# patflick/psac

Hardware: AMD Instinct MI355X
Metric: MChars/s SA+LCP build; rank-pair radix-sort HBM GB/s vs peak (higher is better)
Workload: dtype u64

## Files before the change

include/psacx.h:

```cpp
#ifndef PSACX_H
#define PSACX_H

#include <stddef.h>
#include <stdint.h>

#ifdef __cplusplus
extern "C" {
#endif

typedef struct psacx_ctx psacx_ctx;

enum {
    PSACX_OK = 0,
    PSACX_EINVAL = -1,
    PSACX_ERANGE = -2,
    PSACX_ENOMEM = -3,
    PSACX_EHIP = -4,
    PSACX_EDEVICE = -5,
    PSACX_ENOGPU = -6
};

enum {
    PSACX_LCP = 1u,
    PSACX_NO_FAST = 2u,
// ... 20 lines not shown
    double ms_total;
    double ms_alphabet, ms_kmer, ms_sort_hist, ms_sort_scatter, ms_rebucket, ms_isa_scatter,
           ms_gather, ms_compact, ms_rmq_build, ms_finalize;
    double ms_sort_scatter3, ms_sort_tilehist, ms_sort_scatter2;
    uint64_t scatter_launches[3];
    uint64_t scatter_records[3];
    uint64_t scatter_bytes[3];
    uint64_t hist_bytes;
    uint64_t workspace_bytes;
    uint64_t onew_passes;
    uint64_t heavy_rounds;
    uint64_t heavy_records;
    uint64_t light_records;
    uint64_t level_gathers;
    double ms_host[9];
} psacx_stats;


#define PSACX_STREAM_DEFAULT ((void*)(intptr_t)-1)
int psacx_create(psacx_ctx** out, int device, void* stream);
void psacx_destroy(psacx_ctx* ctx);
const char* psacx_strerror(int code);
const char* psacx_last_hip_error(const psacx_ctx* ctx);
int psacx_trim(psacx_ctx* ctx);

enum {
    PSACX_OPT_RESET = 0, PSACX_OPT_FORCE_DIET, PSACX_OPT_DIET_CAP, PSACX_OPT_ONE_STAGE, PSACX_OPT_TIES_RADIX, PSACX_OPT_NO_ONE_WORD,
    PSACX_OPT_ONE_WORD_ALWAYS, PSACX_OPT_ONE_WORD_MIN, PSACX_OPT_WIDEN_LAST, PSACX_OPT_NO_DIGIT_BYTES, PSACX_OPT_NO_BUCKET_SORT,
    PSACX_OPT_ISA_UPDATE, PSACX_OPT_GATHER, PSACX_OPT_NO_HEAVY, PSACX_OPT_NO_WHOLE, PSACX_OPT_NO_LAZY_RANKS, PSACX_OPT_NO_EARLY_OUT, PSACX_OPT_COUNT
};
int psacx_configure(psacx_ctx* ctx, int option, uint64_t value);
int psacx_configure_from_env(psacx_ctx* ctx);
const char* psacx_debug_env(const char* name);

int psacx_construct_u32(psacx_ctx* ctx, const uint8_t* text, uint64_t n, uint32_t k,
                        uint32_t flags, uint32_t* SA, uint32_t* ISA, uint32_t* LCP);
int psacx_construct_u64(psacx_ctx* ctx, const uint8_t* text, uint64_t n, uint32_t k,
                        uint32_t flags, uint64_t* SA, uint64_t* ISA, uint64_t* LCP);
int psacx_construct_dev_u32(psacx_ctx* ctx, const uint8_t* d_text, uint64_t n, uint32_t k,
                            uint32_t flags, uint32_t* d_SA, uint32_t* d_ISA, uint32_t* d_LCP);
int psacx_construct_dev_u64(psacx_ctx* ctx, const uint8_t* d_text, uint64_t n, uint32_t k,
                            uint32_t flags, uint64_t* d_SA, uint64_t* d_ISA, uint64_t* d_LCP);

int psacx_construct_lc_u32(psacx_ctx* ctx, const uint8_t* text, uint64_t n, uint32_t k, uint32_t flags,
// ... 147 lines not shown
```

psac_amd/_lib.py:

```python
import ctypes as C
import os

_HERE = os.path.dirname(os.path.abspath(__file__))
LIB_PATH = os.path.join(_HERE, "lib", "libpsacx.so")

PSACX_LCP = 1
PSACX_NO_FAST = 2
PSACX_PROFILE = 4
PSACX_MAX_ROUNDS = 72

OPTIONS = {"reset": 0, "force_diet": 1, "diet_cap": 2, "one_stage": 3, "ties_radix": 4, "no_one_word": 5, "one_word_always": 6, "one_word_min": 7,
           "widen_last": 8, "no_digit_bytes": 9, "no_bucket_sort": 10, "isa_update": 11, "gather": 12, "no_heavy": 13, "no_whole": 14, "no_lazy_ranks": 15, "no_early_out": 16}
MULTI_OPTIONS = {"layout": 1, "slab": 2, "output_slack": 3, "trace": 4, "wire_piece": 5, "pieces": 6, "check_chunks": 7, "global_refine_sort": 8,
                 "one_stage": 9, "two_word": 10, "one_word": 11, "no_slices": 12, "slice_wide": 13, "slice_shape": 14}
MULTI_FORCE_WIRE, MULTI_NO_RCCL, MULTI_SHM = 1, 2, 4
ENV_KNOBS = bool(os.environ.get("PSACX_ENV_KNOBS"))
if ENV_KNOBS and os.environ.get("PSACX_LIB"):
    LIB_PATH = os.environ["PSACX_LIB"]

EXPORTS = [
    "psacx_create", "psacx_destroy", "psacx_strerror", "psacx_last_hip_error", "psacx_trim", "psacx_configure", "psacx_configure_from_env", "psacx_debug_env",
    "psacx_construct_u32", "psacx_construct_u64", "psacx_construct_dev_u32", "psacx_construct_dev_u64",
    "psacx_construct_gsa_u32", "psacx_construct_gsa_u64", "psacx_construct_gsa_dev_u32", "psacx_construct_gsa_dev_u64",
    "psacx_construct_lc_u32", "psacx_construct_lc_u64", "psacx_construct_lc_dev_u32", "psacx_construct_lc_dev_u64",
    "psacx_get_stats", "psacx_profile", "psacx_check_dev_u32", "psacx_check_dev_u64", "psacx_check_gsa_dev_u32", "psacx_check_gsa_dev_u64", "psacx_pair_sort_dev_u32", "psacx_pair_sort_dev_u64", "psacx_ansv_u32",
    "psacx_ansv_u64", "psacx_ansv_dev_u32", "psacx_ansv_dev_u64", "psacx_suffix_tree_u32", "psacx_suffix_tree_u64", "psacx_dev_alloc", "psacx_dev_free", "psacx_copy_h2d", "psacx_copy_d2h", "psacx_sync",
    "psacx_rand_dna", "psacx_synth_text_dev",
# ... 13 lines not shown
                ("unfinished_elements", C.c_uint64), ("sort_passes", C.c_uint32),
                ("sort_passes_skipped", C.c_uint32)]


class Stats(C.Structure):
    _fields_ = [("sigma", C.c_uint32), ("bits_per_char", C.c_uint32), ("k", C.c_uint32),
                ("n_rounds", C.c_uint32), ("rounds", Round * PSACX_MAX_ROUNDS),
                ("ms_total", C.c_double), ("ms_alphabet", C.c_double), ("ms_kmer", C.c_double),
                ("ms_sort_hist", C.c_double), ("ms_sort_scatter", C.c_double), ("ms_rebucket", C.c_double),
                ("ms_isa_scatter", C.c_double), ("ms_gather", C.c_double), ("ms_compact", C.c_double),
                ("ms_rmq_build", C.c_double), ("ms_finalize", C.c_double),
                ("ms_sort_scatter3", C.c_double), ("ms_sort_tilehist", C.c_double), ("ms_sort_scatter2", C.c_double),
                ("scatter_launches", C.c_uint64 * 3), ("scatter_records", C.c_uint64 * 3),
                ("scatter_bytes", C.c_uint64 * 3), ("hist_bytes", C.c_uint64), ("workspace_bytes", C.c_uint64), ("onew_passes", C.c_uint64),
                ("heavy_rounds", C.c_uint64), ("heavy_records", C.c_uint64), ("light_records", C.c_uint64), ("level_gathers", C.c_uint64),
                ("ms_host", C.c_double * 9)]


class PsacxError(RuntimeError):
    def __init__(self, code, msg):
        RuntimeError.__init__(self, "psacx error %d: %s" % (code, msg))
        self.code = code


_lib = None


def load():
    global _lib
    if _lib is not None:
        return _lib
# ... 109 lines not shown
```

psac_amd/csrc/construct.hpp:

```cpp
#pragma once
#include <chrono>
#include <thread>
#include "engine.hpp"
#include "bucket_sort.hpp"
#include "heavy_keys.hpp"

namespace psacx {

constexpr int SCAN_ITEMS = 8;
#ifndef RB1W_BLOCK
#define RB1W_BLOCK 512
#endif
template <typename T> struct ScanCfg {
    static constexpr int BLOCK = sizeof(T) == 8 ? 512 : 768;
    static constexpr int TILE = BLOCK * SCAN_ITEMS;
};
constexpr int SCAN_TILE_MIN = 512 * SCAN_ITEMS;

constexpr unsigned SCAN_CHUNKS = 4096, SCAN_CHUNK = 1024 * 4;
template <typename T> struct Work {
    T *bsa;
    SortBufs<T> x, y;
    SortBufs<T> ry;
    T *pos_a, *pos_b;
// ... 571 lines not shown
                               reinterpret_cast<unsigned*>(w.sc.d_desc + 256), (int)lo1);
        } else
            hipLaunchKernelGGL((key_pairs_kernel<T, KB, KI>), dim3((unsigned)nb), dim3(KB), 0, c->stream, d_text, n, n,
                               tab, ks, first_in.k1, k2rec, w.sc.d_partials, (const T*)nullptr);
        PSACX_HIP(c, hipGetLastError());
        PSACX_TRY(summary_finish(c, w.sc, (unsigned)nb));
        return PSACX_OK;
    };
    if (!one_word) PSACX_TRY(make_keys(hist_in_keys));

    std::memset(r0, 0, sizeof(*r0));
    if (two_stage) {
        SortBufs<T> in1{first_in.k1, nullptr, first_in.v}, alt1{first_alt.k1, nullptr, first_alt.v};
        bool packed1 = false;
        uint8_t* tie_bytes = nullptr;
        onew_recs = false;
        if constexpr (sizeof(T) == 8) {
            if (one_word) {
                uint64_t* s1 = nullptr;
                const bool keep = !kn.widen_last && !kn.ties_radix && isa_narrow_levels<T>(n, kn) > 0;
                uint8_t* const dig = kn.no_digit_bytes ? (uint8_t*)nullptr : reinterpret_cast<uint8_t*>(w.diet ? w.x.k2 : first_alt.k2);
                tie_bytes = (keep && !kn.no_digit_bytes) ? reinterpret_cast<uint8_t*>(w.diet ? w.y.k2 : first_in.k2) : (uint8_t*)nullptr;
                const int rc1 = prefix_sort_1w(c, w.sc, reinterpret_cast<uint64_t*>(in1.k1), reinterpret_cast<uint64_t*>(alt1.k1),
                                               reinterpret_cast<uint64_t*>(d_sa), n, lo1, lead, r0, &s1, d_text, n, tab, ks, !kn.one_word_always,
                                               keep ? &onew_view : nullptr, dig,
                                               (in1.k1 == w.x.k1 && onew_pad_total<T>(n)) ? ONEW_PAD : (uint64_t)0, tie_bytes);
                if (rc1 == PSACX_RETRY_1STAGE) {
                    two_stage = false; retry_one_stage = true; one_word = false;
                } else if (rc1 == PSACX_RETRY_1W) {
                    one_word = false;
                    PSACX_TRY(make_keys(hist_in_keys));
                }
                else {
                    PSACX_TRY(rc1);
                    sorted.k1 = reinterpret_cast<T*>(s1); sorted.k2 = nullptr; sorted.v = d_sa;
                    packed1 = true;
                    onew_recs = keep;
                }
            }
        } else one_word = false;
        if (retry_one_stage) continue;
        if (!one_word)
        PSACX_TRY(pair_sort<T>(c, w.sc, in1, alt1, n, true, bits_w1, 0, w.diet ? (T*)nullptr : d_sa, &sorted, r0,
                               ks.spec, n, true, lo1, hist_in_keys ? (int)lo1 : -1));
        if (w.diet && sorted.v != d_sa)
            PSACX_HIP(c, hipMemcpyAsync(d_sa, sorted.v, n * sizeof(T), hipMemcpyDeviceToDevice, c->stream));
        T* S1 = sorted.k1;
        T* const S2 = w.diet ? w.x.k2 : first_alt.k2;
        T* free_k1 = (S1 == w.x.k1) ? w.y.k1 : w.x.k1;
        constexpr int TB = 256, TI = sizeof(T) == 8 ? 32 : 16, TG = 8;
        unsigned long long* d_big = reinterpret_cast<unsigned long long*>(w.d_totals + 2);
        unsigned long long* h_big = reinterpret_cast<unsigned long long*>(c->pinned + 64);
        {
            ProfScope ps(c, TC_GATHER);
            PSACX_HIP(c, hipMemsetAsync(d_big, 0, sizeof(unsigned long long), c->stream));
            const uint64_t nb = (n + (uint64_t)TB * TI - 1) / ((uint64_t)TB * TI);
            if constexpr (sizeof(T) == 8) {
                if (onew_recs)
                    hipLaunchKernelGGL((tie_resolve_1w_kernel<TB, TI, TG>), dim3((unsigned)nb), dim3(TB), 0, c->stream, reinterpret_cast<uint64_t*>(S1),
                                       reinterpret_cast<uint64_t*>(free_k1), reinterpret_cast<uint64_t*>(S2), n, onew_view, d_text, n, tab, ks, d_big,
                                       (const uint8_t*)tie_bytes);
            }
            if (!kn.ties_radix && !onew_recs)
                hipLaunchKernelGGL((tie_resolve_kernel<T, TB, TI, TG>), dim3((unsigned)nb), dim3(TB), 0, c->stream, S1, d_sa, S2, n, lo1,
                                   d_text, n, tab, ks, d_big, packed1);
            PSACX_HIP(c, hipGetLastError());
        }
        PSACX_HIP(c, hipMemcpyAsync(h_big, d_big, sizeof(unsigned long long), hipMemcpyDeviceToHost, c->stream));
        PSACX_HIP(c, hipStreamSynchronize(c->stream));
        if constexpr (sizeof(T) == 8) {
            if (onew_recs && *h_big) {
                ProfScope ps(c, TC_GATHER);
                hipLaunchKernelGGL(onew_widen_kernel<0>, dim3(grid_for(c, n, 256, 8)), dim3(256), 0, c->stream, reinterpret_cast<const uint64_t*>(S1), n, onew_view,
                                   reinterpret_cast<uint64_t*>(free_k1), reinterpret_cast<uint64_t*>(d_sa));
                PSACX_HIP(c, hipGetLastError());
                std::swap(S1, free_k1);
                sorted.k1 = S1;
                onew_recs = false;
            }
        }
        if (*h_big || kn.ties_radix) {
            const uint64_t ntiles = (n + ScanCfg<T>::TILE - 1) / ScanCfg<T>::TILE;
            {
                ProfScope ps(c, TC_COMPACT);
                hipLaunchKernelGGL((count_active_kernel<T, ScanCfg<T>::BLOCK, SCAN_ITEMS>), dim3((unsigned)ntiles), dim3(ScanCfg<T>::BLOCK), 0,
// ... 639 lines not shown
```

psac_amd/csrc/engine.hpp:

```cpp
#pragma once
#include <hip/hip_runtime.h>

#include <algorithm>
#include <cstdio>
#include <cstdlib>
#include <cstring>
#include <condition_variable>
#include <functional>
#include <map>
#include <mutex>
#include <string>
#include <thread>
#include <sched.h>
#include <pthread.h>
#include <cctype>
#include <cstdio>
#include <vector>

#include "../../include/psacx.h"
#include "radix.hpp"
#include "sa_kernels.hpp"

namespace psacx {

// ... 11 lines not shown
    bool force_diet = false;
    uint64_t diet_cap = 0;
    bool one_stage = false;
    bool ties_radix = false;
    bool no_one_word = false;
    bool one_word_always = false;
    unsigned one_word_min = 24;
    int isa_update = 0;
    bool no_digit_bytes = false;
    bool no_bucket_sort = false;
    int gather = 0;
    bool no_heavy = false;
    bool no_early_out = false;
    bool no_lazy_ranks = false;
    bool no_whole = false;
    bool widen_last = false;
};

}

struct psacx_ctx {
    int device = 0;
    hipStream_t stream = nullptr;
    bool own_stream = false;
    char* slab = nullptr;
    size_t slab_bytes = 0;
    char* aux = nullptr;
    size_t aux_bytes = 0;
    char* pinned = nullptr;
    char* pinned_dev = nullptr;
// ... 781 lines not shown
            if (w != dst) PSACX_HIP(c, hipMemcpyAsync(dst, w, n * sizeof(T), hipMemcpyDeviceToDevice, c->stream));
        } else if (dst != cur.v) {
            PSACX_HIP(c, hipMemcpyAsync(dst, cur.v, n * sizeof(T), hipMemcpyDeviceToDevice, c->stream));
        }
        cur.v = dst;
    }
    *res = cur;
    return PSACX_OK;
}

constexpr int PSACX_RETRY_1W = 1001;
constexpr int PSACX_RETRY_1STAGE = 1002;
#ifndef PSACX_1W_ITEMS
#define PSACX_1W_ITEMS 8
#endif
struct OneWordLayout { unsigned slab; uint64_t total_slabs, vtiles; size_t hist_bytes, slab_bytes, tabs_bytes, need; };
template <int TILE>
inline OneWordLayout onew_layout(unsigned long long* h_tabs, uint64_t ntiles_hint) {
    OneWordLayout lay;
    lay.slab = ntiles_hint >= (1u << 16) ? 64u : 16u;
    uint64_t total_slabs = 0;
    for (int d = 0; d < RADIX; ++d) {
        const uint64_t cnt = h_tabs[d + 1] - h_tabs[d];
        h_tabs[RADIX + 1 + d] = total_slabs;
        total_slabs += ((cnt + TILE - 1) / TILE + lay.slab - 1) / lay.slab;
    }
    h_tabs[2 * RADIX + 1] = total_slabs;
    lay.total_slabs = total_slabs;
    lay.vtiles = total_slabs * lay.slab;
    lay.hist_bytes = ((size_t)lay.vtiles * RADIX * sizeof(unsigned) + 255) & ~(size_t)255;
    lay.slab_bytes = ((size_t)total_slabs * RADIX * sizeof(unsigned long long) + 255) & ~(size_t)255;
    lay.tabs_bytes = (2 * (RADIX + 1) * sizeof(unsigned long long) + 64 + total_slabs * sizeof(SlabInfo) + 255) & ~(size_t)255;
    lay.need = 256 + lay.hist_bytes + lay.slab_bytes + (size_t)RADIX * RADIX * 8 + lay.tabs_bytes;
    return lay;
}
inline int onew_bucket_passes(psacx_ctx* c, char* scratch, const unsigned long long* h_tabs, const OneWordLayout& lay, uint64_t* cur, uint64_t* oth, uint64_t* sa_out,
                              unsigned sfield, unsigned low, unsigned lo1, uint64_t nrec, uint64_t** s1, OneWordView* view_out = nullptr, uint8_t* dig = nullptr,
                              uint64_t in_pad = 0, uint8_t* tie_bytes = nullptr) {
    constexpr int BLOCK = 512, ITEMS_B = PSACX_1W_ITEMS, TILE = BLOCK * ITEMS_B;
    unsigned* tile_hist = reinterpret_cast<unsigned*>(scratch + 256);
    unsigned long long* slab_tot = reinterpret_cast<unsigned long long*>(scratch + 256 + lay.hist_bytes);
    unsigned long long* base2 = reinterpret_cast<unsigned long long*>(scratch + 256 + lay.hist_bytes + lay.slab_bytes);
    unsigned long long* d_tabs = base2 + (size_t)RADIX * RADIX;
    OneWordTabs tb;
    tb.bucket_off = d_tabs; tb.slab_start = d_tabs + RADIX + 1; tb.slab = lay.slab;
    SlabInfo* slab_info = reinterpret_cast<SlabInfo*>((reinterpret_cast<uintptr_t>(d_tabs + 2 * (RADIX + 1)) + 31) & ~(uintptr_t)31);
    tb.slab_info = slab_info;
    *s1 = cur;
    if (view_out) { view_out->off = d_tabs; view_out->low = low; view_out->sfield = sfield; view_out->lo1 = lo1; }
    PSACX_HIP(c, hipMemcpyAsync(d_tabs, h_tabs, 2 * (RADIX + 1) * sizeof(unsigned long long), hipMemcpyHostToDevice, c->stream));
    if (lay.total_slabs == 0) return PSACX_OK;
    const uint64_t total_slabs = lay.total_slabs, vtiles = lay.vtiles;
    hipLaunchKernelGGL(radix_slab_info_kernel<0>, dim3((unsigned)((total_slabs + 255) / 256)), dim3(256), 0, c->stream, tb.bucket_off, tb.slab_start,
                       (unsigned)total_slabs, (unsigned)(lay.slab * TILE), slab_info);
    PSACX_HIP(c, hipGetLastError());
    const int npass = (int)((low + RADIX_BITS - 1) / RADIX_BITS);
    for (int j = 0; j < npass; ++j) {
        const bool last = j + 1 == npass;
        const int shift = (int)sfield + j * RADIX_BITS;
        {
            ProfScope ps(c, TC_SORT_TILEHIST);
            if (dig && j > 0) hipLaunchKernelGGL((radix_tile_hist_bytes_kernel<BLOCK, ITEMS_B>), dim3((unsigned)((vtiles + BLOCK / WAVE - 1) / (BLOCK / WAVE))), dim3(BLOCK), 0, c->stream,
                                                 (const uint8_t*)dig, tb, (unsigned)vtiles, tile_hist);
            else
            hipLaunchKernelGGL((radix_tile_hist1w_kernel<BLOCK, ITEMS_B>), dim3((unsigned)vtiles), dim3(BLOCK), 0, c->stream, (const uint64_t*)cur, tb, shift, tile_hist,
                               j == 0 ? in_pad : (uint64_t)0);
            hipLaunchKernelGGL(radix_slab_scan1w_kernel<0>, dim3((unsigned)total_slabs), dim3(RADIX), 0, c->stream, tile_hist, tb, (unsigned)TILE, slab_tot);
            hipLaunchKernelGGL(radix_top_scan1w_kernel<0>, dim3(RADIX), dim3(RADIX), 0, c->stream, slab_tot, tb, base2);
            PSACX_HIP(c, hipGetLastError());
        }
        ProfScope ps(c, TC_SORT_SCATTER2);
        PSACX_HIP(c, hipMemsetAsync(scratch, 0, 256, c->stream));
        if (!last || view_out)
            hipLaunchKernelGGL((radix_scatter1w_kernel<BLOCK, ITEMS_B, 8>), dim3((unsigned)vtiles), dim3(BLOCK), 0, c->stream, (const uint64_t*)cur, oth, (uint64_t*)nullptr, shift,
                               tb, base2, tile_hist, slab_tot, reinterpret_cast<unsigned*>(scratch), sort_chunk_for(nrec, true), 0u,
                               last ? tie_bytes : dig, last ? (int)sfield : shift + RADIX_BITS, j == 0 ? in_pad : (uint64_t)0);
        else {
            hipLaunchKernelGGL((radix_scatter1w_kernel<BLOCK, ITEMS_B, 9>), dim3((unsigned)vtiles), dim3(BLOCK), 0, c->stream, (const uint64_t*)cur, oth, sa_out, shift,
                               tb, base2, tile_hist, slab_tot, reinterpret_cast<unsigned*>(scratch), sort_chunk_for(nrec, true), lo1 | (low << 8) | (sfield << 16),
                               (uint8_t*)nullptr, 0, j == 0 ? in_pad : (uint64_t)0);
        }
        PSACX_HIP(c, hipGetLastError());
        c->stats.scatter_launches[2] += 1; c->stats.scatter_records[2] += nrec; c->stats.scatter_bytes[2] += ((last && !view_out ? 24ull : 16ull) + (((dig && !last) || (last && view_out && tie_bytes)) ? 1ull : 0ull)) * nrec;
        c->stats.onew_passes += 1;
        std::swap(cur, oth);
    }
    *s1 = cur;
    return PSACX_OK;
}
inline int prefix_sort_1w(psacx_ctx* c, SortScratch& sc, uint64_t* k0, uint64_t* a, uint64_t* sa_out, uint64_t n, unsigned lo1, unsigned lead,
                          psacx_round* rs, uint64_t** s1, const uint8_t* text, uint64_t n_text, const CodeTable& tab, const KeyShape& ks, bool probe,
                          OneWordView* view_out = nullptr, uint8_t* dig = nullptr, uint64_t pad = 0, uint8_t* tie_bytes = nullptr) {
    constexpr int BLOCK = 512, ITEMS = 8, TILE0 = BLOCK * ITEMS;
    constexpr int TILE = BLOCK * PSACX_1W_ITEMS;
    const unsigned low = lead - RADIX_BITS;
    const unsigned sfield = 64 - low;
    const uint64_t ntiles = (n + TILE0 - 1) / TILE0;
    char* const scratch = sc.d_desc;
    const unsigned slab0 = slab_tiles_for(ntiles);
    const uint64_t nslabs0 = (ntiles + slab0 - 1) / slab0;
    unsigned* tile_hist0 = reinterpret_cast<unsigned*>(scratch + 256);
    unsigned long long* slab_tot0 = reinterpret_cast<unsigned long long*>(scratch + 256 + ((ntiles * RADIX * sizeof(unsigned) + 255) & ~(size_t)255));
    unsigned long long* base0 = sc.d_base;
    {
        ProfScope ps(c, TC_KMER);
        const uint64_t stride = std::max<uint64_t>(64, n >> 20), samples = n / stride;
        uint64_t slots = 1; while (slots < 4 * samples) slots <<= 1;
// ... 22 lines not shown
    PSACX_HIP(c, hipStreamSynchronize(c->stream));
    unsigned long long* h_tabs = sc.h_base + RADIX;
    for (int d = 0; d < RADIX; ++d) h_tabs[d] = sc.h_base[d];
    h_tabs[RADIX] = n;
    const OneWordLayout lay = onew_layout<TILE>(h_tabs, ntiles);
    if (lay.need > sc.desc_bytes || lay.vtiles >= (1ull << 31)) return PSACX_RETRY_1W;
    {
        ProfScope ps(c, TC_KMER);
        PSACX_HIP(c, hipMemsetAsync(scratch, 0, 256, c->stream));
        hipLaunchKernelGGL((key_scatter1w_kernel<BLOCK, ITEMS>), dim3((unsigned)ntiles), dim3(BLOCK), 0, c->stream, text, n, n_text, tab, ks, pad ? k0 : a, (int)(lo1 + low),
                           base0, tile_hist0, slab_tot0, reinterpret_cast<unsigned*>(scratch), sort_chunk_for(n, true), slab0, lo1 | (sfield << 16), (uint64_t)0,
                           (uint8_t*)nullptr, 0, pad);
        PSACX_HIP(c, hipGetLastError());
    }
    uint64_t* cur = nullptr;
    if (pad) PSACX_TRY(onew_bucket_passes(c, scratch, h_tabs, lay, k0, a, sa_out, sfield, low, lo1, n, &cur, view_out, dig, pad, tie_bytes));
    else PSACX_TRY(onew_bucket_passes(c, scratch, h_tabs, lay, a, k0, sa_out, sfield, low, lo1, n, &cur, view_out, dig, 0, tie_bytes));
    *s1 = cur;
    if (rs) { rs->sort_passes = (uint32_t)((low + RADIX_BITS - 1) / RADIX_BITS + 1); rs->sort_passes_skipped = 0; }
    return PSACX_OK;
}

}
```

psac_amd/csrc/psacx_abi.hip:

```cpp
#include "engine.hpp"

namespace psacx {
int construct_dev_u32(psacx_ctx*, const uint8_t*, uint64_t, uint32_t, uint32_t, uint32_t*, uint32_t*, uint32_t*);
int construct_dev_u64(psacx_ctx*, const uint8_t*, uint64_t, uint32_t, uint32_t, uint64_t*, uint64_t*, uint64_t*);
int construct_host_u32(psacx_ctx*, const uint8_t*, uint64_t, uint32_t, uint32_t, uint32_t*, uint32_t*, uint32_t*);
int construct_gsa_host_u32(psacx_ctx*, const uint8_t*, uint64_t, const uint64_t*, uint64_t, uint32_t, uint32_t, uint32_t*, uint32_t*, uint32_t*);
int construct_gsa_dev_u32(psacx_ctx*, const uint8_t*, uint64_t, const uint64_t*, uint64_t, uint32_t, uint32_t, uint32_t*, uint32_t*, uint32_t*);
int construct_gsa_host_u64(psacx_ctx*, const uint8_t*, uint64_t, const uint64_t*, uint64_t, uint32_t, uint32_t, uint64_t*, uint64_t*, uint64_t*);
int construct_gsa_dev_u64(psacx_ctx*, const uint8_t*, uint64_t, const uint64_t*, uint64_t, uint32_t, uint32_t, uint64_t*, uint64_t*, uint64_t*);
int construct_lc_host_u32(psacx_ctx*, const uint8_t*, uint64_t, uint32_t, uint32_t, uint32_t*, uint32_t*, uint32_t*, uint8_t*);
int construct_lc_host_u64(psacx_ctx*, const uint8_t*, uint64_t, uint32_t, uint32_t, uint64_t*, uint64_t*, uint64_t*, uint8_t*);
int construct_lc_dev_u32(psacx_ctx*, const uint8_t*, uint64_t, uint32_t, uint32_t, uint32_t*, uint32_t*, uint32_t*, uint8_t*);
int construct_lc_dev_u64(psacx_ctx*, const uint8_t*, uint64_t, uint32_t, uint32_t, uint64_t*, uint64_t*, uint64_t*, uint8_t*);
int construct_host_u64(psacx_ctx*, const uint8_t*, uint64_t, uint32_t, uint32_t, uint64_t*, uint64_t*, uint64_t*);
int pair_sort_dev_u32(psacx_ctx*, uint32_t*, uint32_t*, uint32_t*, uint64_t, uint32_t);
int pair_sort_dev_u64(psacx_ctx*, uint64_t*, uint64_t*, uint64_t*, uint64_t, uint32_t);
int check_dev_u32(psacx_ctx*, const uint8_t*, uint64_t, const uint32_t*, const uint32_t*, const uint32_t*, uint64_t*);
int check_dev_u64(psacx_ctx*, const uint8_t*, uint64_t, const uint64_t*, const uint64_t*, const uint64_t*, uint64_t*);
int check_gsa_dev_u32(psacx_ctx*, const uint8_t*, uint64_t, const uint64_t*, uint64_t, const uint32_t*, const uint32_t*, const uint32_t*, uint64_t*);
int check_gsa_dev_u64(psacx_ctx*, const uint8_t*, uint64_t, const uint64_t*, uint64_t, const uint64_t*, const uint64_t*, const uint64_t*, uint64_t*);
int synth_text_dev(psacx_ctx*, uint8_t*, uint64_t, uint64_t, int, uint64_t, uint64_t);
int suffix_tree_host_u32(psacx_ctx*, const uint8_t*, uint64_t, const uint32_t*, const uint32_t*, uint64_t*, uint32_t*);
int suffix_tree_host_u64(psacx_ctx*, const uint8_t*, uint64_t, const uint64_t*, const uint64_t*, uint64_t*, uint32_t*);
int ansv_host_u32(psacx_ctx*, const uint32_t*, uint64_t, int, int, uint64_t, uint64_t*, uint64_t*);
// ... 78 lines not shown
    case PSACX_OPT_DIET_CAP: k.diet_cap = value; return PSACX_OK;
    case PSACX_OPT_ONE_STAGE: k.one_stage = value != 0; return PSACX_OK;
    case PSACX_OPT_TIES_RADIX: k.ties_radix = value != 0; return PSACX_OK;
    case PSACX_OPT_NO_ONE_WORD: k.no_one_word = value != 0; return PSACX_OK;
    case PSACX_OPT_ONE_WORD_ALWAYS: k.one_word_always = value != 0; return PSACX_OK;
    case PSACX_OPT_ONE_WORD_MIN: if (value > 62) return PSACX_EINVAL; k.one_word_min = value ? (unsigned)std::max<uint64_t>(16, value) : 24u; return PSACX_OK;
    case PSACX_OPT_WIDEN_LAST: k.widen_last = value != 0; return PSACX_OK;
    case PSACX_OPT_NO_DIGIT_BYTES: k.no_digit_bytes = value != 0; return PSACX_OK;
    case PSACX_OPT_NO_BUCKET_SORT: k.no_bucket_sort = value != 0; return PSACX_OK;
    case PSACX_OPT_ISA_UPDATE: if (value > 2) return PSACX_EINVAL; k.isa_update = (int)value; return PSACX_OK;
    case PSACX_OPT_GATHER: if (value > 2) return PSACX_EINVAL; k.gather = (int)value; return PSACX_OK;
    case PSACX_OPT_NO_HEAVY: k.no_heavy = value != 0; return PSACX_OK;
    case PSACX_OPT_NO_WHOLE: k.no_whole = value != 0; return PSACX_OK;
    case PSACX_OPT_NO_LAZY_RANKS: k.no_lazy_ranks = value != 0; return PSACX_OK;
    case PSACX_OPT_NO_EARLY_OUT: k.no_early_out = value != 0; return PSACX_OK;
    default: return PSACX_EINVAL;
    }
}

const char* psacx_debug_env(const char* name) { return name ? getenv(name) : nullptr; }

int psacx_configure_from_env(psacx_ctx* c) {
    if (!c) return PSACX_EINVAL;
    static const struct { const char* name; int option; } flags[] = {
        {"PSACX_FORCE_DIET", PSACX_OPT_FORCE_DIET}, {"PSACX_ONE_STAGE", PSACX_OPT_ONE_STAGE}, {"PSACX_TIES_RADIX", PSACX_OPT_TIES_RADIX},
        {"PSACX_NO_ONE_WORD", PSACX_OPT_NO_ONE_WORD}, {"PSACX_ONE_WORD_ALWAYS", PSACX_OPT_ONE_WORD_ALWAYS}, {"PSACX_WIDEN_LAST", PSACX_OPT_WIDEN_LAST},
        {"PSACX_NO_DIGIT_BYTES", PSACX_OPT_NO_DIGIT_BYTES}, {"PSACX_NO_BUCKET_SORT", PSACX_OPT_NO_BUCKET_SORT}, {"PSACX_NO_HEAVY", PSACX_OPT_NO_HEAVY},
        {"PSACX_NO_WHOLE", PSACX_OPT_NO_WHOLE}, {"PSACX_NO_LAZY_RANKS", PSACX_OPT_NO_LAZY_RANKS},
        {"PSACX_NO_EARLY_OUT", PSACX_OPT_NO_EARLY_OUT}};
    (void)psacx_configure(c, PSACX_OPT_RESET, 0);
    for (const auto& f : flags) if (psacx_debug_env(f.name)) (void)psacx_configure(c, f.option, 1);
    if (const char* e = psacx_debug_env("PSACX_DIET_CAP")) (void)psacx_configure(c, PSACX_OPT_DIET_CAP, strtoull(e, nullptr, 10));
    if (const char* e = psacx_debug_env("PSACX_ONE_WORD_MIN")) (void)psacx_configure(c, PSACX_OPT_ONE_WORD_MIN, strtoull(e, nullptr, 10));
    if (const char* e = psacx_debug_env("PSACX_ISA_UPDATE")) (void)psacx_configure(c, PSACX_OPT_ISA_UPDATE, e[0] == 's' ? 1 : 2);
    if (const char* e = psacx_debug_env("PSACX_GATHER")) (void)psacx_configure(c, PSACX_OPT_GATHER, e[0] == 'f' ? 1 : 2);
    return PSACX_OK;
}

int psacx_trim(psacx_ctx* c) {
    if (!c) return PSACX_EINVAL;
    PSACX_HIP(c, hipSetDevice(c->device));
    PSACX_HIP(c, hipStreamSynchronize(c->stream));
    if (c->slab) { PSACX_HIP(c, hipFree(c->slab)); c->slab = nullptr; c->slab_bytes = 0; }
    if (c->aux) { PSACX_HIP(c, hipFree(c->aux)); c->aux = nullptr; c->aux_bytes = 0; }
    if (c->io) { PSACX_HIP(c, hipFree(c->io)); c->io = nullptr; c->io_bytes = 0; }
    if (c->dstage) { PSACX_HIP(c, hipFree(c->dstage)); c->dstage = nullptr; }
    for (int i = 0; i < psacx_ctx::STAGE_SLOTS; ++i) {
// ... 145 lines not shown
```

psac_amd/csrc/sa_kernels.hpp:

```cpp
#pragma once
#ifndef RB_WAVES_ATTR
#define RB_WAVES_ATTR
#endif
#ifndef RB_ABLATE
#define RB_ABLATE 0
#endif
#include <type_traits>
#include "dev_common.hpp"

namespace psacx {

constexpr int RADIX_P = 256;

struct CodeTable { uint16_t c[256]; };

template <typename T>
__device__ __forceinline__ void key_summary_add(unsigned long long* partials, T or1, T and1, T or2, T and2) {
    __shared__ unsigned long long red[4][16];
    or1 = wave_reduce<T>(or1, OpOr()); and1 = wave_reduce<T>(and1, OpAnd());
    or2 = wave_reduce<T>(or2, OpOr()); and2 = wave_reduce<T>(and2, OpAnd());
    const unsigned wave = threadIdx.x / WAVE, nw = (blockDim.x + WAVE - 1) / WAVE;
    const unsigned long long hi = ~(unsigned long long)(T)~(T)0;
    if (lane_id() == 0) {
        red[0][wave] = (unsigned long long)or1; red[1][wave] = (unsigned long long)and1 | hi;
// ... 1518 lines not shown
        }
        unsigned rank = 0;
#pragma unroll
        for (int j = 0; j < G; ++j) {
            const T o1 = shfl<T>(k1, (int)(seg0 + j)), o2 = shfl<T>(k2, (int)(seg0 + j));
            if (o1 < k1 || (o1 == k1 && (o2 < k2 || (o2 == k2 && (unsigned)j < m)))) ++rank;
        }
        const bool moved = ((unsigned)(__ballot(member && rank != m) >> seg0) & ((1u << G) - 1u)) != 0;
        if (member) {
            W1[e + rank] = k1; S2[e + rank] = k2;
            if (moved) R[e + rank] = (key << ow.sfield) | sa;
        }
    }
}

template <typename T, int BLOCK>
__global__ __launch_bounds__(BLOCK) void gather_prefix_ties_kernel(uint64_t cnt, T* __restrict__ K1, const T* __restrict__ V,
                                          const uint8_t* __restrict__ text, uint64_t n_text, CodeTable tab, KeyShape ks,
                                          T* __restrict__ K2, unsigned long long* __restrict__ summary, bool packed = false,
                                          const uint32_t* __restrict__ ord = nullptr, unsigned lo1 = 0, int v32 = 0) {
    __shared__ uint16_t ctab[256];
    for (int i = threadIdx.x; i < 256; i += BLOCK) ctab[i] = tab.c[i];
    __syncthreads();
    const uint64_t stride = (uint64_t)gridDim.x * blockDim.x;
    const T lowmask = lo1 ? (T)(((T)1 << lo1) - 1) : (T)0;
    T o1 = 0, a1 = ~(T)0, o2 = 0, a2 = ~(T)0;
    for (uint64_t j = (uint64_t)blockIdx.x * blockDim.x + threadIdx.x; j < cnt; j += stride) {
        T k1 = K1[j], k2;
        const uint64_t sa = v32 ? (uint64_t)reinterpret_cast<const uint32_t*>(V)[j] : (uint64_t)V[j];
        if (packed && ord) window_low_and_word2<T>(text, n_text, ctab, ks, sa, k1, lo1, k1, k2);
// ... 548 lines not shown
```

Baseline: 24730.

## Skip last one-word radix pass and order short runs locally in tie kernel

In the one-word prefix sort, the final (lowest) radix digit pass is skipped when local ordering is enabled. Records sharing the higher digits are instead ordered inside a new tile-local kernel that insertion-sorts short runs in shared memory and fuses this with tie resolution. Runs that are too long are appended to a list and sorted by a separate per-run counting-sort kernel. The goal is to save one full global scatter pass over the records. In exchange it adds a host round trip for the long-run count, and falls back to a one-stage retry if the list overflows its cap.

```diff
diff --git a/include/psacx.h b/include/psacx.h
--- a/include/psacx.h
+++ b/include/psacx.h
@@ -58,6 +58,8 @@
     uint64_t light_records;
     uint64_t level_gathers;
     double ms_host[9];
+    uint64_t local_long_runs;
+    uint64_t local_list_overflows;
 } psacx_stats;
 
 
@@ -71,7 +73,8 @@
 enum {
     PSACX_OPT_RESET = 0, PSACX_OPT_FORCE_DIET, PSACX_OPT_DIET_CAP, PSACX_OPT_ONE_STAGE, PSACX_OPT_TIES_RADIX, PSACX_OPT_NO_ONE_WORD,
     PSACX_OPT_ONE_WORD_ALWAYS, PSACX_OPT_ONE_WORD_MIN, PSACX_OPT_WIDEN_LAST, PSACX_OPT_NO_DIGIT_BYTES, PSACX_OPT_NO_BUCKET_SORT,
-    PSACX_OPT_ISA_UPDATE, PSACX_OPT_GATHER, PSACX_OPT_NO_HEAVY, PSACX_OPT_NO_WHOLE, PSACX_OPT_NO_LAZY_RANKS, PSACX_OPT_NO_EARLY_OUT, PSACX_OPT_COUNT
+    PSACX_OPT_ISA_UPDATE, PSACX_OPT_GATHER, PSACX_OPT_NO_HEAVY, PSACX_OPT_NO_WHOLE, PSACX_OPT_NO_LAZY_RANKS, PSACX_OPT_NO_EARLY_OUT,
+    PSACX_OPT_NO_LOCAL_ORDER, PSACX_OPT_LOCAL_LIST_CAP, PSACX_OPT_COUNT
 };
 int psacx_configure(psacx_ctx* ctx, int option, uint64_t value);
 int psacx_configure_from_env(psacx_ctx* ctx);
diff --git a/psac_amd/_lib.py b/psac_amd/_lib.py
--- a/psac_amd/_lib.py
+++ b/psac_amd/_lib.py
@@ -10,7 +10,8 @@
 PSACX_MAX_ROUNDS = 72
 
 OPTIONS = {"reset": 0, "force_diet": 1, "diet_cap": 2, "one_stage": 3, "ties_radix": 4, "no_one_word": 5, "one_word_always": 6, "one_word_min": 7,
-           "widen_last": 8, "no_digit_bytes": 9, "no_bucket_sort": 10, "isa_update": 11, "gather": 12, "no_heavy": 13, "no_whole": 14, "no_lazy_ranks": 15, "no_early_out": 16}
+           "widen_last": 8, "no_digit_bytes": 9, "no_bucket_sort": 10, "isa_update": 11, "gather": 12, "no_heavy": 13, "no_whole": 14, "no_lazy_ranks": 15, "no_early_out": 16,
+           "no_local_order": 17, "local_list_cap": 18}
 MULTI_OPTIONS = {"layout": 1, "slab": 2, "output_slack": 3, "trace": 4, "wire_piece": 5, "pieces": 6, "check_chunks": 7, "global_refine_sort": 8,
                  "one_stage": 9, "two_word": 10, "one_word": 11, "no_slices": 12, "slice_wide": 13, "slice_shape": 14}
 MULTI_FORCE_WIRE, MULTI_NO_RCCL, MULTI_SHM = 1, 2, 4
@@ -54,7 +55,7 @@
                 ("scatter_launches", C.c_uint64 * 3), ("scatter_records", C.c_uint64 * 3),
                 ("scatter_bytes", C.c_uint64 * 3), ("hist_bytes", C.c_uint64), ("workspace_bytes", C.c_uint64), ("onew_passes", C.c_uint64),
                 ("heavy_rounds", C.c_uint64), ("heavy_records", C.c_uint64), ("light_records", C.c_uint64), ("level_gathers", C.c_uint64),
-                ("ms_host", C.c_double * 9)]
+                ("ms_host", C.c_double * 9), ("local_long_runs", C.c_uint64), ("local_list_overflows", C.c_uint64)]
 
 
 class PsacxError(RuntimeError):
diff --git a/psac_amd/csrc/construct.hpp b/psac_amd/csrc/construct.hpp
--- a/psac_amd/csrc/construct.hpp
+++ b/psac_amd/csrc/construct.hpp
@@ -609,6 +609,7 @@
         SortBufs<T> in1{first_in.k1, nullptr, first_in.v}, alt1{first_alt.k1, nullptr, first_alt.v};
         bool packed1 = false;
         uint8_t* tie_bytes = nullptr;
+        OneWordLocal local;
         onew_recs = false;
         if constexpr (sizeof(T) == 8) {
             if (one_word) {
@@ -616,10 +617,12 @@
                 const bool keep = !kn.widen_last && !kn.ties_radix && isa_narrow_levels<T>(n, kn) > 0;
                 uint8_t* const dig = kn.no_digit_bytes ? (uint8_t*)nullptr : reinterpret_cast<uint8_t*>(w.diet ? w.x.k2 : first_alt.k2);
                 tie_bytes = (keep && !kn.no_digit_bytes) ? reinterpret_cast<uint8_t*>(w.diet ? w.y.k2 : first_in.k2) : (uint8_t*)nullptr;
+                local.on = keep && !kn.no_local_order; local.cap = kn.local_list_cap;
                 const int rc1 = prefix_sort_1w(c, w.sc, reinterpret_cast<uint64_t*>(in1.k1), reinterpret_cast<uint64_t*>(alt1.k1),
                                                reinterpret_cast<uint64_t*>(d_sa), n, lo1, lead, r0, &s1, d_text, n, tab, ks, !kn.one_word_always,
                                                keep ? &onew_view : nullptr, dig,
-                                               (in1.k1 == w.x.k1 && onew_pad_total<T>(n)) ? ONEW_PAD : (uint64_t)0, tie_bytes);
+                                               (in1.k1 == w.x.k1 && onew_pad_total<T>(n)) ? ONEW_PAD : (uint64_t)0, tie_bytes, &local);
+                if (rc1 != PSACX_OK) local.on = false;
                 if (rc1 == PSACX_RETRY_1STAGE) {
                     two_stage = false; retry_one_stage = true; one_word = false;
                 } else if (rc1 == PSACX_RETRY_1W) {
@@ -644,14 +647,19 @@
         T* const S2 = w.diet ? w.x.k2 : first_alt.k2;
         T* free_k1 = (S1 == w.x.k1) ? w.y.k1 : w.x.k1;
         constexpr int TB = 256, TI = sizeof(T) == 8 ? 32 : 16, TG = 8;
+        constexpr int LO_BLOCK = 256, LO_ITEMS = 16, LO_RUN_MAX = 32;
         unsigned long long* d_big = reinterpret_cast<unsigned long long*>(w.d_totals + 2);
         unsigned long long* h_big = reinterpret_cast<unsigned long long*>(c->pinned + 64);
         {
             ProfScope ps(c, TC_GATHER);
-            PSACX_HIP(c, hipMemsetAsync(d_big, 0, sizeof(unsigned long long), c->stream));
+            PSACX_HIP(c, hipMemsetAsync(d_big, 0, 2 * sizeof(unsigned long long), c->stream));
             const uint64_t nb = (n + (uint64_t)TB * TI - 1) / ((uint64_t)TB * TI);
             if constexpr (sizeof(T) == 8) {
-                if (onew_recs)
+                if (onew_recs && local.on)
+                    hipLaunchKernelGGL((local_order_tie_1w_kernel<LO_BLOCK, LO_ITEMS, TG, LO_RUN_MAX>), dim3((unsigned)((n + LO_BLOCK * LO_ITEMS - 1) / (LO_BLOCK * LO_ITEMS))),
+                                       dim3(LO_BLOCK), 0, c->stream, reinterpret_cast<uint64_t*>(S1), reinterpret_cast<uint64_t*>(free_k1), reinterpret_cast<uint64_t*>(S2),
+                                       n, onew_view, d_text, n, tab, ks, d_big, local.list, local.cap);
+                else if (onew_recs)
                     hipLaunchKernelGGL((tie_resolve_1w_kernel<TB, TI, TG>), dim3((unsigned)nb), dim3(TB), 0, c->stream, reinterpret_cast<uint64_t*>(S1),
                                        reinterpret_cast<uint64_t*>(free_k1), reinterpret_cast<uint64_t*>(S2), n, onew_view, d_text, n, tab, ks, d_big,
                                        (const uint8_t*)tie_bytes);
@@ -661,9 +669,30 @@
                                    d_text, n, tab, ks, d_big, packed1);
             PSACX_HIP(c, hipGetLastError());
         }
-        PSACX_HIP(c, hipMemcpyAsync(h_big, d_big, sizeof(unsigned long long), hipMemcpyDeviceToHost, c->stream));
+        PSACX_HIP(c, hipMemcpyAsync(h_big, d_big, 2 * sizeof(unsigned long long), hipMemcpyDeviceToHost, c->stream));
         PSACX_HIP(c, hipStreamSynchronize(c->stream));
         if constexpr (sizeof(T) == 8) {
+            if (onew_recs && local.on && h_big[1]) {
+                c->stats.local_long_runs += h_big[1];
+                if (h_big[1] > local.cap) {
+                    c->stats.local_list_overflows += 1;
+                    two_stage = false; retry_one_stage = true; onew_recs = false;
+                    continue;
+                }
+                ProfScope ps(c, TC_GATHER);
+                const unsigned runs = (unsigned)h_big[1];
+                hipLaunchKernelGGL((local_order_long_kernel<256>), dim3(std::min(runs, 4096u)), dim3(256), 0, c->stream, reinterpret_cast<uint64_t*>(S1),
+                                   reinterpret_cast<uint64_t*>(free_k1), onew_view, local.list, runs);
+                if (!*h_big) {
+                    const uint64_t nb = (n + (uint64_t)TB * TI - 1) / ((uint64_t)TB * TI);
+                    hipLaunchKernelGGL((tie_resolve_1w_kernel<TB, TI, TG>), dim3((unsigned)nb), dim3(TB), 0, c->stream, reinterpret_cast<uint64_t*>(S1),
+                                       reinterpret_cast<uint64_t*>(free_k1), reinterpret_cast<uint64_t*>(S2), n, onew_view, d_text, n, tab, ks, d_big,
+                                       (const uint8_t*)nullptr);
+                }
+                PSACX_HIP(c, hipGetLastError());
+                PSACX_HIP(c, hipMemcpyAsync(h_big, d_big, sizeof(unsigned long long), hipMemcpyDeviceToHost, c->stream));
+                PSACX_HIP(c, hipStreamSynchronize(c->stream));
+            }
             if (onew_recs && *h_big) {
                 ProfScope ps(c, TC_GATHER);
                 hipLaunchKernelGGL(onew_widen_kernel<0>, dim3(grid_for(c, n, 256, 8)), dim3(256), 0, c->stream, reinterpret_cast<const uint64_t*>(S1), n, onew_view,
diff --git a/psac_amd/csrc/engine.hpp b/psac_amd/csrc/engine.hpp
--- a/psac_amd/csrc/engine.hpp
+++ b/psac_amd/csrc/engine.hpp
@@ -49,6 +49,8 @@
     bool no_early_out = false;
     bool no_lazy_ranks = false;
     bool no_whole = false;
+    bool no_local_order = false;
+    unsigned local_list_cap = 0;
     bool widen_last = false;
 };
 
@@ -860,6 +862,7 @@
 #ifndef PSACX_1W_ITEMS
 #define PSACX_1W_ITEMS 8
 #endif
+struct OneWordLocal { bool on = false; unsigned long long* list = nullptr; unsigned cap = 0; };
 struct OneWordLayout { unsigned slab; uint64_t total_slabs, vtiles; size_t hist_bytes, slab_bytes, tabs_bytes, need; };
 template <int TILE>
 inline OneWordLayout onew_layout(unsigned long long* h_tabs, uint64_t ntiles_hint) {
@@ -882,7 +885,7 @@
 }
 inline int onew_bucket_passes(psacx_ctx* c, char* scratch, const unsigned long long* h_tabs, const OneWordLayout& lay, uint64_t* cur, uint64_t* oth, uint64_t* sa_out,
                               unsigned sfield, unsigned low, unsigned lo1, uint64_t nrec, uint64_t** s1, OneWordView* view_out = nullptr, uint8_t* dig = nullptr,
-                              uint64_t in_pad = 0, uint8_t* tie_bytes = nullptr) {
+                              uint64_t in_pad = 0, uint8_t* tie_bytes = nullptr, bool local_order = false) {
     constexpr int BLOCK = 512, ITEMS_B = PSACX_1W_ITEMS, TILE = BLOCK * ITEMS_B;
     unsigned* tile_hist = reinterpret_cast<unsigned*>(scratch + 256);
     unsigned long long* slab_tot = reinterpret_cast<unsigned long long*>(scratch + 256 + lay.hist_bytes);
@@ -900,10 +903,11 @@
     hipLaunchKernelGGL(radix_slab_info_kernel<0>, dim3((unsigned)((total_slabs + 255) / 256)), dim3(256), 0, c->stream, tb.bucket_off, tb.slab_start,
                        (unsigned)total_slabs, (unsigned)(lay.slab * TILE), slab_info);
     PSACX_HIP(c, hipGetLastError());
-    const int npass = (int)((low + RADIX_BITS - 1) / RADIX_BITS);
+    const int skip = local_order ? 1 : 0;
+    const int npass = (int)((low + RADIX_BITS - 1) / RADIX_BITS) - skip;
     for (int j = 0; j < npass; ++j) {
         const bool last = j + 1 == npass;
-        const int shift = (int)sfield + j * RADIX_BITS;
+        const int shift = (int)sfield + (j + skip) * RADIX_BITS;
         {
             ProfScope ps(c, TC_SORT_TILEHIST);
             if (dig && j > 0) hipLaunchKernelGGL((radix_tile_hist_bytes_kernel<BLOCK, ITEMS_B>), dim3((unsigned)((vtiles + BLOCK / WAVE - 1) / (BLOCK / WAVE))), dim3(BLOCK), 0, c->stream,
@@ -920,14 +924,14 @@
         if (!last || view_out)
             hipLaunchKernelGGL((radix_scatter1w_kernel<BLOCK, ITEMS_B, 8>), dim3((unsigned)vtiles), dim3(BLOCK), 0, c->stream, (const uint64_t*)cur, oth, (uint64_t*)nullptr, shift,
                                tb, base2, tile_hist, slab_tot, reinterpret_cast<unsigned*>(scratch), sort_chunk_for(nrec, true), 0u,
-                               last ? tie_bytes : dig, last ? (int)sfield : shift + RADIX_BITS, j == 0 ? in_pad : (uint64_t)0);
+                               last ? (local_order ? (uint8_t*)nullptr : tie_bytes) : dig, last ? (int)sfield : shift + RADIX_BITS, j == 0 ? in_pad : (uint64_t)0);
         else {
             hipLaunchKernelGGL((radix_scatter1w_kernel<BLOCK, ITEMS_B, 9>), dim3((unsigned)vtiles), dim3(BLOCK), 0, c->stream, (const uint64_t*)cur, oth, sa_out, shift,
                                tb, base2, tile_hist, slab_tot, reinterpret_cast<unsigned*>(scratch), sort_chunk_for(nrec, true), lo1 | (low << 8) | (sfield << 16),
                                (uint8_t*)nullptr, 0, j == 0 ? in_pad : (uint64_t)0);
         }
         PSACX_HIP(c, hipGetLastError());
-        c->stats.scatter_launches[2] += 1; c->stats.scatter_records[2] += nrec; c->stats.scatter_bytes[2] += ((last && !view_out ? 24ull : 16ull) + (((dig && !last) || (last && view_out && tie_bytes)) ? 1ull : 0ull)) * nrec;
+        c->stats.scatter_launches[2] += 1; c->stats.scatter_records[2] += nrec; c->stats.scatter_bytes[2] += ((last && !view_out ? 24ull : 16ull) + (((dig && !last) || (last && view_out && tie_bytes && !local_order)) ? 1ull : 0ull)) * nrec;
         c->stats.onew_passes += 1;
         std::swap(cur, oth);
     }
@@ -936,7 +940,7 @@
 }
 inline int prefix_sort_1w(psacx_ctx* c, SortScratch& sc, uint64_t* k0, uint64_t* a, uint64_t* sa_out, uint64_t n, unsigned lo1, unsigned lead,
                           psacx_round* rs, uint64_t** s1, const uint8_t* text, uint64_t n_text, const CodeTable& tab, const KeyShape& ks, bool probe,
-                          OneWordView* view_out = nullptr, uint8_t* dig = nullptr, uint64_t pad = 0, uint8_t* tie_bytes = nullptr) {
+                          OneWordView* view_out = nullptr, uint8_t* dig = nullptr, uint64_t pad = 0, uint8_t* tie_bytes = nullptr, OneWordLocal* local = nullptr) {
     constexpr int BLOCK = 512, ITEMS = 8, TILE0 = BLOCK * ITEMS;
     constexpr int TILE = BLOCK * PSACX_1W_ITEMS;
     const unsigned low = lead - RADIX_BITS;
@@ -989,8 +993,14 @@
         PSACX_HIP(c, hipGetLastError());
     }
     uint64_t* cur = nullptr;
-    if (pad) PSACX_TRY(onew_bucket_passes(c, scratch, h_tabs, lay, k0, a, sa_out, sfield, low, lo1, n, &cur, view_out, dig, pad, tie_bytes));
-    else PSACX_TRY(onew_bucket_passes(c, scratch, h_tabs, lay, a, k0, sa_out, sfield, low, lo1, n, &cur, view_out, dig, 0, tie_bytes));
+    const bool lo = local && local->on && view_out && low >= 2 * RADIX_BITS && low % RADIX_BITS == 0 && n <= (1ull << low);
+    if (local) {
+        local->on = lo;
+        local->list = reinterpret_cast<unsigned long long*>(scratch + 256);
+        local->cap = (unsigned)std::min<uint64_t>(local->cap ? local->cap : 8192u, lay.hist_bytes / sizeof(unsigned long long));
+    }
+    if (pad) PSACX_TRY(onew_bucket_passes(c, scratch, h_tabs, lay, k0, a, sa_out, sfield, low, lo1, n, &cur, view_out, dig, pad, tie_bytes, lo));
+    else PSACX_TRY(onew_bucket_passes(c, scratch, h_tabs, lay, a, k0, sa_out, sfield, low, lo1, n, &cur, view_out, dig, 0, tie_bytes, lo));
     *s1 = cur;
     if (rs) { rs->sort_passes = (uint32_t)((low + RADIX_BITS - 1) / RADIX_BITS + 1); rs->sort_passes_skipped = 0; }
     return PSACX_OK;
diff --git a/psac_amd/csrc/psacx_abi.hip b/psac_amd/csrc/psacx_abi.hip
--- a/psac_amd/csrc/psacx_abi.hip
+++ b/psac_amd/csrc/psacx_abi.hip
@@ -116,6 +116,8 @@
     case PSACX_OPT_NO_WHOLE: k.no_whole = value != 0; return PSACX_OK;
     case PSACX_OPT_NO_LAZY_RANKS: k.no_lazy_ranks = value != 0; return PSACX_OK;
     case PSACX_OPT_NO_EARLY_OUT: k.no_early_out = value != 0; return PSACX_OK;
+    case PSACX_OPT_NO_LOCAL_ORDER: k.no_local_order = value != 0; return PSACX_OK;
+    case PSACX_OPT_LOCAL_LIST_CAP: if (value > (1u << 20)) return PSACX_EINVAL; k.local_list_cap = (unsigned)value; return PSACX_OK;
     default: return PSACX_EINVAL;
     }
 }
@@ -129,10 +131,11 @@
         {"PSACX_NO_ONE_WORD", PSACX_OPT_NO_ONE_WORD}, {"PSACX_ONE_WORD_ALWAYS", PSACX_OPT_ONE_WORD_ALWAYS}, {"PSACX_WIDEN_LAST", PSACX_OPT_WIDEN_LAST},
         {"PSACX_NO_DIGIT_BYTES", PSACX_OPT_NO_DIGIT_BYTES}, {"PSACX_NO_BUCKET_SORT", PSACX_OPT_NO_BUCKET_SORT}, {"PSACX_NO_HEAVY", PSACX_OPT_NO_HEAVY},
         {"PSACX_NO_WHOLE", PSACX_OPT_NO_WHOLE}, {"PSACX_NO_LAZY_RANKS", PSACX_OPT_NO_LAZY_RANKS},
-        {"PSACX_NO_EARLY_OUT", PSACX_OPT_NO_EARLY_OUT}};
+        {"PSACX_NO_EARLY_OUT", PSACX_OPT_NO_EARLY_OUT}, {"PSACX_NO_LOCAL_ORDER", PSACX_OPT_NO_LOCAL_ORDER}};
     (void)psacx_configure(c, PSACX_OPT_RESET, 0);
     for (const auto& f : flags) if (psacx_debug_env(f.name)) (void)psacx_configure(c, f.option, 1);
     if (const char* e = psacx_debug_env("PSACX_DIET_CAP")) (void)psacx_configure(c, PSACX_OPT_DIET_CAP, strtoull(e, nullptr, 10));
+    if (const char* e = psacx_debug_env("PSACX_LOCAL_LIST_CAP")) (void)psacx_configure(c, PSACX_OPT_LOCAL_LIST_CAP, strtoull(e, nullptr, 10));
     if (const char* e = psacx_debug_env("PSACX_ONE_WORD_MIN")) (void)psacx_configure(c, PSACX_OPT_ONE_WORD_MIN, strtoull(e, nullptr, 10));
     if (const char* e = psacx_debug_env("PSACX_ISA_UPDATE")) (void)psacx_configure(c, PSACX_OPT_ISA_UPDATE, e[0] == 's' ? 1 : 2);
     if (const char* e = psacx_debug_env("PSACX_GATHER")) (void)psacx_configure(c, PSACX_OPT_GATHER, e[0] == 'f' ? 1 : 2);
diff --git a/psac_amd/csrc/sa_kernels.hpp b/psac_amd/csrc/sa_kernels.hpp
--- a/psac_amd/csrc/sa_kernels.hpp
+++ b/psac_amd/csrc/sa_kernels.hpp
@@ -1556,6 +1556,189 @@
     }
 }
 
+constexpr int LOCAL_HALO = 64;
+template <int BLOCK, int ITEMS, int G, int LB>
+__global__ __launch_bounds__(BLOCK) void local_order_tie_1w_kernel(uint64_t* R, uint64_t* __restrict__ W1, uint64_t* __restrict__ S2,
+                                                                   uint64_t n, OneWordView ow, const uint8_t* __restrict__ text, uint64_t n_text,
+                                                                   CodeTable tab, KeyShape ks, unsigned long long* __restrict__ big,
+                                                                   unsigned long long* __restrict__ long_list, unsigned long_cap) {
+    typedef uint64_t T;
+    constexpr int TILE = BLOCK * ITEMS, NQ = TILE + LOCAL_HALO, NWORD = NQ / 64;
+    static_assert(ITEMS % 2 == 0 && BLOCK % WAVE == 0 && WAVE == 64 && BLOCK >= LOCAL_HALO, "pairs of records per thread, one flag word per wave");
+    static_assert(LB >= 16 && LB < LOCAL_HALO && NQ < 65536 && G == 8, "a run that starts in the tile ends inside the halo; eight lanes per group");
+    __shared__ uint16_t ctab[256];
+    __shared__ unsigned long long s_off[257];
+    __shared__ __attribute__((aligned(16))) T s_rec[NQ];
+    __shared__ unsigned long long s_start[NWORD + 1];
+    __shared__ unsigned groups[TILE / 2 + LB];
+    __shared__ unsigned n_groups;
+    __shared__ T s_before;
+    const unsigned tid = threadIdx.x, lane = lane_id();
+    for (int i = tid; i < 256; i += BLOCK) ctab[i] = tab.c[i];
+    for (int i = tid; i < 257; i += BLOCK) s_off[i] = ow.off[i];
+    const uint64_t t0 = (uint64_t)blockIdx.x * TILE;
+    if (tid == 0) { n_groups = 0; s_start[NWORD] = 0; s_before = t0 ? R[t0 - 1] : (T)0; }
+    T P[ITEMS + 2];
+    auto load_pair = [&](unsigned q, T& a, T& b) {
+        const uint64_t e = t0 + q;
+        a = 0; b = 0;
+        if (e + 1 < n) { const ulonglong2 v = *reinterpret_cast<const ulonglong2*>(R + e); a = v.x; b = v.y; }
+        else if (e < n) a = R[e];
+        *reinterpret_cast<ulonglong2*>(s_rec + q) = make_ulonglong2(a, b);
+    };
+#pragma unroll
+    for (int k = 0; k < ITEMS / 2; ++k) load_pair(2u * ((unsigned)k * BLOCK + tid), P[2 * k], P[2 * k + 1]);
+    P[ITEMS] = 0; P[ITEMS + 1] = 0;
+    if (tid < LOCAL_HALO / 2) load_pair((unsigned)TILE + 2u * tid, P[ITEMS], P[ITEMS + 1]);
+    __syncthreads();
+    ow.off = s_off;
+    const unsigned sf = ow.sfield, hs = ow.sfield + 8;
+    const unsigned b0 = onew_bucket(ow, t0);
+    const uint64_t first_start = s_off[b0], next_start = s_off[b0 + 1];
+    for (int k = 0; k <= ITEMS; ++k) {
+        if (k == ITEMS && tid >= (unsigned)LOCAL_HALO) break;
+        const unsigned q = (unsigned)k * BLOCK + tid;
+        const uint64_t e = t0 + q;
+        bool st = true;
+        if (e < n && e != 0) {
+            const T x = s_rec[q], pv = q ? s_rec[q - 1] : s_before;
+            st = (x >> hs) != (pv >> hs) || e == first_start || (e >= next_start && s_off[onew_bucket(ow, e)] == e);
+        }
+        const unsigned long long m = __ballot(st);
+        if (lane == 0) s_start[q >> 6] = m;
+    }
+    __syncthreads();
+    for (int k = 0; k < ITEMS; ++k) {
+        const unsigned q = (unsigned)k * BLOCK + tid;
+        const uint64_t e = t0 + q;
+        if (e >= n || !((s_start[q >> 6] >> (q & 63u)) & 1ull)) continue;
+        const unsigned q1 = q + 1, w1 = q1 >> 6, sh1 = q1 & 63u;
+        unsigned long long win = s_start[w1] >> sh1;
+        if (sh1) win |= s_start[w1 + 1] << (64u - sh1);
+        if (win & 1ull) continue;
+        const unsigned len = win ? (unsigned)__builtin_ctzll(win) + 1u : (unsigned)LOCAL_HALO + 1u;
+        if (len > (unsigned)LB) {
+            const unsigned long long at = atomicAdd(&big[1], 1ull);
+            if (at < long_cap) long_list[at] = e;
+            continue;
+        }
+        for (unsigned i = 1; i < len; ++i) {
+            const T v = s_rec[q + i];
+            const unsigned dv = (unsigned)(v >> sf) & 255u;
+            unsigned j = i;
+            while (j > 0) {
+                const T u = s_rec[q + j - 1];
+                if (((unsigned)(u >> sf) & 255u) <= dv) break;
+                s_rec[q + j] = u;
+                --j;
+            }
+            if (j != i) s_rec[q + j] = v;
+        }
+        unsigned gs = 0, dp = (unsigned)(s_rec[q] >> sf) & 255u;
+        for (unsigned i = 1; i <= len; ++i) {
+            const unsigned d = i < len ? (unsigned)(s_rec[q + i] >> sf) & 255u : 256u;
+            if (d != dp) {
+                if (i - gs >= 2) groups[atomicAdd(&n_groups, 1u)] = (q + gs) | ((i - gs) << 16);
+                gs = i; dp = d;
+            }
+        }
+    }
+    __syncthreads();
+    const unsigned ng = __hip_atomic_load(big, __ATOMIC_RELAXED, __HIP_MEMORY_SCOPE_AGENT) ? 0u : n_groups;
+    const T smask = (1ull << sf) - 1;
+    const unsigned m = lane & (G - 1), seg0 = lane & ~(unsigned)(G - 1);
+    for (unsigned g0 = 0; g0 < ng; g0 += BLOCK / G) {
+        const unsigned g = g0 + tid / G;
+        const bool live = g < ng;
+        const unsigned gd = live ? groups[g] : 0u, q = gd & 0xffffu, glen = gd >> 16;
+        const uint64_t e = t0 + q;
+        const bool too_long = glen > (unsigned)G;
+        const bool member = live && !too_long && m < glen;
+        if (live && too_long && m == 0) atomicAdd(big, 1ull);
+        const T rec = member ? s_rec[q + m] : (T)0;
+        const T sa = rec & smask;
+        T k1 = ~(T)0, k2 = ~(T)0;
+        if (member) window_low_and_word2<T>(text, n_text, ctab, ks, sa, (T)onew_word1(ow, onew_bucket(ow, e), rec), ow.lo1, k1, k2);
+        unsigned rank = 0;
+#pragma unroll
+        for (int j = 0; j < G; ++j) {
+            const T o1 = shfl<T>(k1, (int)(seg0 + j)), o2 = shfl<T>(k2, (int)(seg0 + j));
+            if (o1 < k1 || (o1 == k1 && (o2 < k2 || (o2 == k2 && (unsigned)j < m)))) ++rank;
+        }
+        if (member) {
+            W1[e + rank] = k1; S2[e + rank] = k2;
+            if (rank != m) s_rec[q + rank] = rec;
+        }
+    }
+    __syncthreads();
+    auto store_pair = [&](unsigned q, T a0, T b0) {
+        const uint64_t e = t0 + q;
+        const ulonglong2 v = *reinterpret_cast<const ulonglong2*>(s_rec + q);
+        const bool ca = v.x != a0, cb = v.y != b0;
+        if (ca && cb) *reinterpret_cast<ulonglong2*>(R + e) = v;
+        else if (ca) R[e] = v.x;
+        else if (cb) R[e + 1] = v.y;
+    };
+#pragma unroll
+    for (int k = 0; k < ITEMS / 2; ++k) store_pair(2u * ((unsigned)k * BLOCK + tid), P[2 * k], P[2 * k + 1]);
+    if (tid < LOCAL_HALO / 2) store_pair((unsigned)TILE + 2u * tid, P[ITEMS], P[ITEMS + 1]);
+}
+
+template <int BLOCK>
+__global__ __launch_bounds__(BLOCK) void local_order_long_kernel(uint64_t* R, uint64_t* __restrict__ tmp, OneWordView ow,
+                                                                 const unsigned long long* __restrict__ long_list, unsigned runs) {
+    typedef uint64_t T;
+    static_assert(BLOCK == 256, "one thread per digit value");
+    __shared__ unsigned long long cnt[256], base[256];
+    __shared__ unsigned short sd[BLOCK];
+    __shared__ unsigned long long s_end;
+    const unsigned tid = threadIdx.x, sf = ow.sfield, hs = ow.sfield + 8;
+    for (unsigned r = blockIdx.x; r < runs; r += gridDim.x) {
+        const uint64_t rs = long_list[r];
+        const uint64_t bend = ow.off[onew_bucket(ow, rs) + 1];
+        const T hi = R[rs] >> hs;
+        if (tid == 0) s_end = bend;
+        cnt[tid] = 0;
+        __syncthreads();
+        for (uint64_t c0 = rs + 1; c0 < bend; c0 += BLOCK) {
+            const uint64_t i = c0 + tid;
+            if (i < bend && (R[i] >> hs) != hi) atomicMin(&s_end, (unsigned long long)i);
+            __syncthreads();
+            const bool found = s_end != bend;
+            __syncthreads();
+            if (found) break;
+        }
+        const uint64_t re = s_end;
+        for (uint64_t i = rs + tid; i < re; i += BLOCK) atomicAdd(&cnt[(unsigned)(R[i] >> sf) & 255u], 1ull);
+        __syncthreads();
+        unsigned long long sum = 0;
+        for (unsigned d = 0; d < tid; ++d) sum += cnt[d];
+        base[tid] = sum;
+        __syncthreads();
+        for (uint64_t c0 = rs; c0 < re; c0 += BLOCK) {
+            const uint64_t i = c0 + tid;
+            const bool act = i < re;
+            const T rec = act ? R[i] : (T)0;
+            const unsigned d = act ? (unsigned)(rec >> sf) & 255u : 0xffffu;
+            sd[tid] = (unsigned short)d;
+            __syncthreads();
+            unsigned before = 0, total = 0;
+            for (unsigned j = 0; j < (unsigned)BLOCK; ++j) {
+                const unsigned same = sd[j] == d ? 1u : 0u;
+                total += same;
+                before += j < tid ? same : 0u;
+            }
+            const unsigned long long pos = act ? base[d] + before : 0ull;
+            if (act) tmp[rs + pos] = rec;
+            __syncthreads();
+            if (act && before + 1 == total) base[d] = pos + 1;
+            __syncthreads();
+        }
+        for (uint64_t i = rs + tid; i < re; i += BLOCK) R[i] = tmp[i];
+        __syncthreads();
+    }
+}
+
 template <typename T, int BLOCK>
 __global__ __launch_bounds__(BLOCK) void gather_prefix_ties_kernel(uint64_t cnt, T* __restrict__ K1, const T* __restrict__ V,
                                           const uint8_t* __restrict__ text, uint64_t n_text, CodeTable tab, KeyShape ks,
```

Result: slower. 19620 (-20.7%).
